# Biogod2020/Spatial-Clip

Hardware: AMD Instinct MI355X
Metric: tile-gene pairs/sec (train step) (higher is better)
Workload: dtype bf16

## Files before the change

### spatial-clip_amd/csrc/sc_gemm8p.hip

```cpp
#include "sc_gemm_common.h"
#include <stdlib.h>
#include <map>
#include <mutex>

namespace {

constexpr int BM = 256, BN = 256, BK = 64;
constexpr int HALF = 128 * 64 * 2;
constexpr int RING = 8 * HALF;
constexpr int EPI_BYTES = 8 * 64 * SC_EPI_LD * 4;
constexpr int LDS_BYTES = EPI_BYTES > RING ? EPI_BYTES : RING;

typedef const __attribute__((address_space(1))) void* gptr_t;
typedef __attribute__((address_space(3))) void* lptr_t;

SC_DEVICE void dma16(const void* src, char* lds_wave_base) {
    __builtin_amdgcn_global_load_lds((gptr_t)src, (lptr_t)lds_wave_base, 16, 0, 0);
}

template <int EPI, bool Q8 = false, bool LUT = false>
SC_DEVICE void epilogue_bf16_lds(f32x4 (&acc)[8][4], const GemmArgs& g, char* strip, int row0, int col0, int lane,
                                 const unsigned* lut = nullptr) {
    float amax_lane = 0.f;
    const float q8s = (Q8 && sc_epi_gelu_fwd(EPI) && g.q8) ? *g.q8_scale : 0.f;
    const int li = lane & 15, lg = lane >> 4;
    constexpr bool kBias = (EPI == SC_EPI_BF16_BIAS || sc_epi_gelu_fwd(EPI));
    f32x4 bj[4];
#pragma unroll
    for (int j = 0; j < 4; ++j) {
        bj[j] = (f32x4){0.f, 0.f, 0.f, 0.f};
        const int c = col0 + j * 16 + lg * 4;
        if (kBias && g.bias && c < g.N) bj[j] = *reinterpret_cast<const f32x4*>(g.bias + c);
    }
    bf16* C = reinterpret_cast<bf16*>(g.C);
    bf16* C2 = reinterpret_cast<bf16*>(g.C2);
    const int rr = lane >> 3, rc = lane & 7;
    const int gcol = col0 + rc * 8;
#pragma unroll
    for (int p = 0; p < 4; ++p) {
#pragma unroll
        for (int ib = 0; ib < 2; ++ib) {
            const int r = ib * 16 + li;
#pragma unroll
            for (int j = 0; j < 4; ++j) {
                const f32x4 v = acc[p * 2 + ib][j] + bj[j];
                const int chunk = (j * 2 + (lg >> 1)) ^ (r & 7);
                *reinterpret_cast<u32x2*>(strip + r * 128 + chunk * 16 + (lg & 1) * 8) = sc_pack4(v[0], v[1], v[2], v[3]);
            }
        }
        __builtin_amdgcn_s_waitcnt(0xC07F);
        __builtin_amdgcn_wave_barrier();
#pragma unroll
        for (int s4 = 0; s4 < 4; ++s4) {
            const int r = s4 * 8 + rr;
            const u32x4 u = *reinterpret_cast<const u32x4*>(strip + r * 128 + ((rc ^ (r & 7)) << 4));
            const int grow = row0 + p * 32 + r;
            if (grow < g.M && gcol < g.N) {
                if (EPI != SC_EPI_GELU_GRAD_PAIR) *reinterpret_cast<u32x4*>(C + (size_t)grow * g.ldc + gcol) = u;
                if (sc_epi_gelu_fwd(EPI)) {
                    union { u32x4 w; bf16x8 h; } x;
                    x.w = u;
                    bf16x8 o;
                    if (EPI == SC_EPI_GELU_PAIR) {
#pragma unroll
                        for (int e = 0; e < 8; ++e) o[e] = (bf16)sc_act((float)x.h[e], g.act);
                    } else {
                        bf16x8 gd;
                        bool formula = true;
                        if (LUT) {
                            unsigned ent[8];
                            bool inside = true;
#pragma unroll
                            for (int e = 0; e < 8; ++e) {
                                const unsigned bits = (u[e >> 1] >> ((e & 1) * 16)) & 0xFFFFu;
                                const unsigned rel = (bits & 0x7FFFu) - (unsigned)SC_GELU_LUT_LO;
                                inside = inside && rel < (unsigned)SC_GELU_LUT_HALF;
                                const unsigned idx = min(rel, (unsigned)SC_GELU_LUT_HALF - 1u) + (bits >> 15) * (unsigned)SC_GELU_LUT_HALF;
                                ent[e] = lut[idx];
                            }
                            formula = __builtin_amdgcn_ballot_w64(!inside) != 0;
                            if (!formula) {
                                union { u32x4 w; bf16x8 h; } lo, hi;
#pragma unroll
                                for (int q = 0; q < 4; ++q) {
                                    lo.w[q] = __builtin_amdgcn_perm(ent[2 * q + 1], ent[2 * q], 0x05040100u);
                                    hi.w[q] = __builtin_amdgcn_perm(ent[2 * q + 1], ent[2 * q], 0x07060302u);
                                }
                                o = lo.h;
                                gd = hi.h;
                            }
                        }
                        if (formula) {
#pragma unroll
                            for (int e = 0; e < 8; ++e) {
                                float hv, gv;
                                sc_act_both((float)x.h[e], g.act, hv, gv);
                                o[e] = (bf16)hv;
                                gd[e] = (bf16)gv;
                            }
                        }
                        *reinterpret_cast<bf16x8*>(C + (size_t)grow * g.ldc + gcol) = gd;
                    }
                    *reinterpret_cast<bf16x8*>(C2 + (size_t)grow * g.ldc2 + gcol) = o;
                    if (Q8 && g.q8) {
                        float r[8];
#pragma unroll
                        for (int e = 0; e < 8; ++e) { r[e] = (float)o[e]; amax_lane = fmaxf(amax_lane, fabsf(r[e])); }
                        *reinterpret_cast<u32x2*>(g.q8 + (size_t)grow * g.ldq8 + gcol) = sc_pack8_fp8(r, q8s);
                    }
                }
            }
        }
        __builtin_amdgcn_s_waitcnt(0xC07F);
        __builtin_amdgcn_wave_barrier();
    }
    if (Q8 && sc_epi_gelu_fwd(EPI) && g.q8) sc_amax_publish(amax_lane, g.q8_amax);
}

constexpr int slot(int D, int q) { return D * 4 * HALF + q * HALF; }

struct Stager {
    const bf16* src[4][2];
    int nt;
    int wave;
};

template <int D, int PH>
SC_DEVICE void phase(char* smem, const Stager& S, int t, const int (&a_off)[2], const int (&b_off)[2], bf16x8 (&a)[8],
                     bf16x8 (&b0)[4], bf16x8 (&b1)[4], f32x4 (&acc)[8][4]) {
    if (PH == 1) {
#pragma unroll
        for (int kk = 0; kk < 2; ++kk)
#pragma unroll
            for (int jj = 0; jj < 2; ++jj)
                b0[kk * 2 + jj] = *reinterpret_cast<const bf16x8*>(smem + slot(D, 1) + b_off[kk] + jj * 2048);
    }
    if (PH == 2) {
#pragma unroll
        for (int kk = 0; kk < 2; ++kk)
#pragma unroll
            for (int jj = 0; jj < 2; ++jj)
                b1[kk * 2 + jj] = *reinterpret_cast<const bf16x8*>(smem + slot(D, 2) + b_off[kk] + jj * 2048);
    }
    if (PH == 1 || PH == 3) {
        constexpr int sl = slot(D, PH == 1 ? 0 : 3);
#pragma unroll
        for (int kk = 0; kk < 2; ++kk)
#pragma unroll
            for (int ii = 0; ii < 4; ++ii)
                a[kk * 4 + ii] = *reinterpret_cast<const bf16x8*>(smem + sl + a_off[kk] + ii * 2048);
    }
    constexpr int q = (PH + 1) & 3;
    constexpr int DS = PH <= 2 ? (D ^ 1) : D;
    const int ts = t + (PH <= 2 ? 1 : 2);
    if (ts < S.nt) {
        dma16(S.src[q][0] + (size_t)ts * BK, smem + slot(DS, q) + S.wave * 1024);
        dma16(S.src[q][1] + (size_t)ts * BK, smem + slot(DS, q) + (8 + S.wave) * 1024);
        asm volatile("s_waitcnt vmcnt(8)" ::: "memory");
    } else {
        asm volatile("s_waitcnt vmcnt(0)" ::: "memory");
    }
    __builtin_amdgcn_sched_barrier(0);
    __builtin_amdgcn_s_barrier();
    __builtin_amdgcn_sched_barrier(0);
    constexpr int mi = PH >= 3 ? 1 : 0;
    constexpr int nj = (PH == 2 || PH == 3) ? 1 : 0;
    __builtin_amdgcn_s_setprio(1);
#pragma unroll
    for (int kk = 0; kk < 2; ++kk)
#pragma unroll
        for (int ii = 0; ii < 4; ++ii)
#pragma unroll
            for (int jj = 0; jj < 2; ++jj)
                acc[mi * 4 + ii][nj * 2 + jj] =
                    sc_mfma16(nj ? b1[kk * 2 + jj] : b0[kk * 2 + jj], a[kk * 4 + ii], acc[mi * 4 + ii][nj * 2 + jj]);
    __builtin_amdgcn_s_setprio(0);
    __builtin_amdgcn_sched_barrier(0);
    __builtin_amdgcn_s_barrier();
    __builtin_amdgcn_sched_barrier(0);
}

template <int D>
SC_DEVICE void ktile(char* smem, const Stager& S, int t, const int (&a_off)[2], const int (&b_off)[2], bf16x8 (&a)[8],
                     bf16x8 (&b0)[4], bf16x8 (&b1)[4], f32x4 (&acc)[8][4]) {
    phase<D, 1>(smem, S, t, a_off, b_off, a, b0, b1, acc);
    phase<D, 2>(smem, S, t, a_off, b_off, a, b0, b1, acc);
    phase<D, 3>(smem, S, t, a_off, b_off, a, b0, b1, acc);
    phase<D, 4>(smem, S, t, a_off, b_off, a, b0, b1, acc);
}

template <int EPI>
__global__ __launch_bounds__(512, 2) void gemm8p_kernel(const GemmArgs g) {
    extern __shared__ __attribute__((aligned(16))) char smem[];
    const int t = threadIdx.x;
    const int lane = t & 63;
    const int wave = __builtin_amdgcn_readfirstlane(t >> 6);
    const int wr = wave >> 2, wc = wave & 3;
    const int li = lane & 15, lg = lane >> 4;

    int idx = sc_xcd_remap(blockIdx.x, gridDim.x);
    int tn, tm, z;
    if (g.col_group > 0) {
        sc_tile_colgroup(idx, g, tm, tn);
        z = 0;
    } else {
        tn = idx % g.ntn;
        idx /= g.ntn;
        tm = idx % g.ntm;
        z = idx / g.ntm;
    }
    const int m0 = tm * BM, n0 = tn * BN;
    const int kbeg = z * g.k_per_split;
    const int kend = min(g.K, kbeg + g.k_per_split);

    Stager S;
    S.nt = (kend - kbeg) / BK;
    S.wave = wave;
#pragma unroll
    for (int p = 0; p < 2; ++p) {
        const int r = (p * 8 + wave) * 8 + (lane >> 3);
        const int lc = (lane & 7) ^ ((r >> 1) & 7);
#pragma unroll
        for (int h = 0; h < 2; ++h) {
            const int ga = min(m0 + (r >> 6) * 128 + h * 64 + (r & 63), g.M - 1);
            const int gb = min(n0 + (r >> 5) * 64 + h * 32 + (r & 31), g.N - 1);
            S.src[h ? 3 : 0][p] = g.A + (size_t)ga * g.lda + kbeg + lc * 8;
            S.src[h ? 2 : 1][p] = g.B + (size_t)gb * g.ldb + kbeg + lc * 8;
        }
    }
    int a_off[2], b_off[2];
#pragma unroll
    for (int kk = 0; kk < 2; ++kk) {
        const int coff = ((kk * 4 + lg) ^ ((li >> 1) & 7)) << 4;
        a_off[kk] = (wr * 64 + li) * 128 + coff;
        b_off[kk] = (wc * 32 + li) * 128 + coff;
    }

    f32x4 acc[8][4];
#pragma unroll
    for (int i = 0; i < 8; ++i)
#pragma unroll
        for (int j = 0; j < 4; ++j) acc[i][j] = (f32x4){0.f, 0.f, 0.f, 0.f};

#pragma unroll
    for (int s = 0; s < 6; ++s) {
        const int ts = s >> 2, q = s & 3;
        if (ts < S.nt) {
            dma16(S.src[q][0] + (size_t)ts * BK, smem + slot(ts & 1, q) + wave * 1024);
            dma16(S.src[q][1] + (size_t)ts * BK, smem + slot(ts & 1, q) + (8 + wave) * 1024);
        }
    }
    if (S.nt > 1) asm volatile("s_waitcnt vmcnt(8)" ::: "memory");
    else asm volatile("s_waitcnt vmcnt(0)" ::: "memory");
    __builtin_amdgcn_sched_barrier(0);
    __builtin_amdgcn_s_barrier();
    if (wr == 1) __builtin_amdgcn_s_barrier();
    __builtin_amdgcn_sched_barrier(0);

    bf16x8 a[8], b0[4], b1[4];
    for (int kt = 0; kt < S.nt; kt += 2) {
        ktile<0>(smem, S, kt, a_off, b_off, a, b0, b1, acc);
        if (kt + 1 < S.nt) ktile<1>(smem, S, kt + 1, a_off, b_off, a, b0, b1, acc);
    }
    if (wr == 0) __builtin_amdgcn_s_barrier();
    asm volatile("s_waitcnt vmcnt(0)" ::: "memory");
    __builtin_amdgcn_sched_barrier(0);

    if (EPI == SC_EPI_GELU_GRAD_PAIR && g.gelu_lut != nullptr) {
        unsigned* lut = reinterpret_cast<unsigned*>(smem + 8 * 4096);
        for (int c = t; c < SC_GELU_LUT_N / 4; c += 512)
            reinterpret_cast<u32x4*>(lut)[c] = reinterpret_cast<const u32x4*>(g.gelu_lut)[c];
        __syncthreads();
        epilogue_bf16_lds<EPI, false, true>(acc, g, smem + wave * 4096, m0 + wr * 128, n0 + wc * 64, lane, lut);
    } else if (EPI == SC_EPI_BF16 || EPI == SC_EPI_BF16_BIAS || sc_epi_gelu_fwd(EPI)) {
        epilogue_bf16_lds<EPI>(acc, g, smem + wave * 4096, m0 + wr * 128, n0 + wc * 64, lane);
    } else {
        const int mw = wr * 128;
        float* ep = reinterpret_cast<float*>(smem) + wave * 64 * SC_EPI_LD;
        EpiRegs<EPI> er;
        sc_epi_load<EPI>(er, m0 + mw, n0 + wc * 64, lane, g, 64);
#pragma unroll
        for (int h = 0; h < 2; ++h) {
#pragma unroll
            for (int i = 0; i < 4; ++i)
#pragma unroll
                for (int j = 0; j < 4; ++j) sc_epi_put(ep, i, j, li, lg, acc[h * 4 + i][j]);
            __builtin_amdgcn_s_waitcnt(0xC07F);
            __builtin_amdgcn_wave_barrier();
            sc_epilogue_store<EPI>(ep, er, m0 + mw + h * 64, n0 + wc * 64, lane, g, z, (h + 1 < 2) ? m0 + mw + 64 : -1, 64);
            __builtin_amdgcn_s_waitcnt(0xC07F);
            __builtin_amdgcn_wave_barrier();
        }
    }
}

__global__ void sc_gelu_lut_fill_kernel(unsigned* lut, int act) {
    const int i = blockIdx.x * blockDim.x + threadIdx.x;
    if (i >= SC_GELU_LUT_N) return;
    const unsigned bits = (unsigned)(SC_GELU_LUT_LO + i % SC_GELU_LUT_HALF) | (i >= SC_GELU_LUT_HALF ? 0x8000u : 0u);
    const float u = __uint_as_float(bits << 16);
    float hv, gv;
    sc_act_both(u, act, hv, gv);
    union { bf16 b; unsigned short s; } h, gq;
    h.b = (bf16)hv;
    gq.b = (bf16)gv;
    lut[i] = ((unsigned)gq.s << 16) | (unsigned)h.s;
}

template <int EPI>
int launch(const GemmArgs& g, int nblocks, hipStream_t st) {
    static bool attr_done = false;
    if (!attr_done) {
        (void)hipFuncSetAttribute(reinterpret_cast<const void*>(&gemm8p_kernel<EPI>),
                                  hipFuncAttributeMaxDynamicSharedMemorySize, LDS_BYTES);
        attr_done = true;
    }
    gemm8p_kernel<EPI><<<nblocks, 512, LDS_BYTES, st>>>(g);
    SC_LAUNCH_CHECK();
    return 1;
}


enum { PW_STEADY = 0, PW_POSTEPI = 1, PW_DRAIN0 = 2 };

struct PStager {
    const bf16* src[4][2];
    long long koff;
    int sk;
    int stile;
    int nt, wave, total, stride;
};

SC_DEVICE void pstage_set_tile(PStager& S, const GemmArgs& g, int lane) {
    const int tn = S.stile % g.ntn, tm = S.stile / g.ntn;
    const int m0 = tm * BM, n0 = tn * BN;
#pragma unroll
    for (int p = 0; p < 2; ++p) {
        const int r = (p * 8 + S.wave) * 8 + (lane >> 3);
        const int lc = (lane & 7) ^ ((r >> 1) & 7);
#pragma unroll
        for (int h = 0; h < 2; ++h) {
            const int ga = min(m0 + (r >> 6) * 128 + h * 64 + (r & 63), g.M - 1);
            const int gb = min(n0 + (r >> 5) * 64 + h * 32 + (r & 31), g.N - 1);
            S.src[h ? 3 : 0][p] = g.A + (size_t)ga * g.lda + lc * 8;
            S.src[h ? 2 : 1][p] = g.B + (size_t)gb * g.ldb + lc * 8;
        }
    }
}
SC_DEVICE void pstage_advance(PStager& S, const GemmArgs& g, int lane) {
    S.sk += 1;
    S.koff += BK;
    if (S.sk == S.nt) {
        S.sk = 0;
        S.koff = 0;
        S.stile += S.stride;
        if (S.stile < S.total) pstage_set_tile(S, g, lane);
    }
}

template <int PH, int ESTORES>
SC_DEVICE void pphase(char* smem, int doff, PStager& S, const GemmArgs& g, int lane, int pw, const int (&a_off)[2],
                      const int (&b_off)[2], bf16x8 (&a)[8], bf16x8 (&b0)[4], bf16x8 (&b1)[4], f32x4 (&acc)[8][4]) {
    const char* cur = smem + doff;
    if (PH == 1) {
#pragma unroll
        for (int kk = 0; kk < 2; ++kk)
#pragma unroll
            for (int jj = 0; jj < 2; ++jj)
                b0[kk * 2 + jj] = *reinterpret_cast<const bf16x8*>(cur + 1 * HALF + b_off[kk] + jj * 2048);
    }
// ... 855 lines not shown
    int total = 0;
    for (int p = 0; p < n; ++p) {
        gg.g[p] = g[p];
        gg.first[p] = total;
        total += g[p].ntm * g[p].ntn * g[p].splitk;
    }
    for (int p = n; p <= SC_WGRAD_GROUP_MAX; ++p) gg.first[p] = total;
    static bool attr_done = false;
    if (!attr_done) {
        (void)hipFuncSetAttribute(reinterpret_cast<const void*>(&gemm8p_tn_group_kernel),
                                  hipFuncAttributeMaxDynamicSharedMemorySize, LDS_BYTES);
        attr_done = true;
    }
    gemm8p_tn_group_kernel<<<total, 512, LDS_BYTES, st>>>(gg);
    SC_LAUNCH_CHECK();
    return 1;
}

int sc_gemm8p_tn_fp8(GemmArgs& g, int splitk_req, float* slabs, hipStream_t st) {
    if (g.M < 256 || g.N < 192 || (g.K % 128) != 0 || (g.M % 16) != 0 || (g.N % 16) != 0) return 0;
    if ((g.lda % 16) != 0 || (g.ldb % 16) != 0) return 0;
    g.ntm = (g.M + BM - 1) / BM;
    g.ntn = (g.N + BN - 1) / BN;
    const int ktiles = g.K / 128;
    int splitk = splitk_req < 1 ? 1 : splitk_req;
    if (slabs == nullptr) splitk = 1;
    if (splitk > ktiles) splitk = ktiles;
    const int tiles_per = (ktiles + splitk - 1) / splitk;
    splitk = (ktiles + tiles_per - 1) / tiles_per;
    g.splitk = splitk;
    g.k_per_split = tiles_per * 128;
    g.slab_stride = 0;
    if (splitk > 1) {
        if (g.ldc != g.N) return 0;
        g.C = slabs;
        g.slab_stride = (long long)g.M * g.N;
    }
    static bool attr_done = false;
    if (!attr_done) {
        (void)hipFuncSetAttribute(reinterpret_cast<const void*>(&gemm8p_tn_f8_kernel), hipFuncAttributeMaxDynamicSharedMemorySize,
                                  LDS_BYTES);
        attr_done = true;
    }
    gemm8p_tn_f8_kernel<<<g.ntm * g.ntn * splitk, 512, LDS_BYTES, st>>>(g);
    SC_LAUNCH_CHECK();
    return 1;
}

static int sc_colgroup_default(int epi, const GemmArgs& g) {
    (void)epi; (void)g;
    return 0;
}

int sc_gemm8p_try(int mode, int epi, GemmArgs& g, int splitk_req, float* slabs, hipStream_t st) {
    if (g.M < 256 || g.N < 192 || (g.K % BK) != 0) return 0;
    if (mode == SC_GEMM_TN && (epi != SC_EPI_F32 || (g.M % 8) != 0 || (g.N % 8) != 0)) return 0;
    if ((long long)g.M * g.N < 256LL * 256 * 8) return 0;
    if (mode == SC_GEMM_NT && splitk_req <= 1) {
        static const int small_tiles = getenv("SC_GEMM_SMALL_TILES") ? atoi(getenv("SC_GEMM_SMALL_TILES")) : 100;
        if ((long long)g.M * g.N < 256LL * 256 * small_tiles) return 0;
    }
    g.ntm = (g.M + BM - 1) / BM;
    g.ntn = (g.N + BN - 1) / BN;
    const int ktiles = g.K / BK;
    int splitk = splitk_req < 1 ? 1 : splitk_req;
    if (epi != SC_EPI_F32 || slabs == nullptr) splitk = 1;
    if (splitk > ktiles) splitk = ktiles;
    int tiles_per = (ktiles + splitk - 1) / splitk;
    splitk = (ktiles + tiles_per - 1) / tiles_per;
    g.splitk = splitk;
    g.k_per_split = tiles_per * BK;
    g.slab_stride = 0;
    if (splitk > 1) {
        if (g.ldc != g.N) return 0;
        g.C = slabs;
        g.slab_stride = (long long)g.M * g.N;
    }
    const int nblocks = g.ntm * g.ntn * splitk;
    if (mode == SC_GEMM_TN) {
        return launch_tn(g, nblocks, st);
    }
    if (epi == SC_EPI_GELU_GRAD_PAIR) {
        const char* sw = getenv("SC_GELU_LUT");
        if (!(sw && sw[0] == '0')) g.gelu_lut = sc_gelu_lut_device(st, g.act);
    }
    static const bool persist = !(getenv("SC_GEMM_PERSIST") && getenv("SC_GEMM_PERSIST")[0] == '0');
    if (g.gelu_lut == nullptr && persist && splitk == 1 && nblocks >= 1024 && ktiles >= 3) {
        if (epi == SC_EPI_BF16) return launch_persistent<SC_EPI_BF16>(g, nblocks, st);
        if (epi == SC_EPI_BF16_BIAS) return launch_persistent<SC_EPI_BF16_BIAS>(g, nblocks, st);
        if (epi == SC_EPI_GELU_PAIR) return launch_persistent<SC_EPI_GELU_PAIR>(g, nblocks, st);
        if (epi == SC_EPI_GELU_GRAD_PAIR) return launch_persistent<SC_EPI_GELU_GRAD_PAIR>(g, nblocks, st);
    }
    g.col_group = 0;
    if (splitk == 1 && g.ntn > 1) {
        int gc = sc_colgroup_default(epi, g);
        if (const char* sw = getenv("SC_GEMM_COLGROUP")) {
            for (const char* p = sw; *p;) {
                char* e = nullptr;
                const long ep = strtol(p, &e, 10);
                if (e == p || *e != ':') break;
                const long v = strtol(e + 1, &e, 10);
                if (ep == epi || ep == -1) gc = (int)v;
                p = (*e == ',') ? e + 1 : e;
                if (*e != ',') break;
            }
        }
        if (gc > 0 && gc < g.ntn) {
            g.col_group = gc;
            g.band_rows = (g.ntm + 7) / 8;
        }
    }
    int rc = 0;
#define SC_CASE(EPI) \
    if (epi == EPI) rc = launch<EPI>(g, nblocks, st);
    SC_CASE(SC_EPI_BF16)
    SC_CASE(SC_EPI_BF16_BIAS)
    SC_CASE(SC_EPI_F32_BIAS_RES)
    SC_CASE(SC_EPI_GELU_PAIR)
    SC_CASE(SC_EPI_BF16_DGELU)
    SC_CASE(SC_EPI_F32)
    SC_CASE(SC_EPI_BF16_BIAS_RES)
    SC_CASE(SC_EPI_GELU_GRAD_PAIR)
    SC_CASE(SC_EPI_BF16_MUL_AUX)
#undef SC_CASE
    return rc;
}

const unsigned* sc_gelu_lut_device(hipStream_t st, int act) {
    static std::mutex mu;
    static std::map<int, unsigned*> all;
    int dev = 0;
    if (hipGetDevice(&dev) != hipSuccess) return nullptr;
    const int key = dev * 2 + (act ? 1 : 0);
    std::lock_guard<std::mutex> lock(mu);
    auto it = all.find(key);
    if (it != all.end()) return it->second;
    unsigned* p = nullptr;
    if (hipMalloc(reinterpret_cast<void**>(&p), SC_GELU_LUT_N * sizeof(unsigned)) != hipSuccess) p = nullptr;
    if (p) {
        sc_gelu_lut_fill_kernel<<<(SC_GELU_LUT_N + 255) / 256, 256, 0, st>>>(p, act ? 1 : 0);
        if (hipGetLastError() != hipSuccess || hipStreamSynchronize(st) != hipSuccess) {
            (void)hipFree(p);
            p = nullptr;
        }
    }
    all[key] = p;
    return p;
}
```

### spatial-clip_amd/csrc/sc_gemm_common.h

```cpp
#pragma once
#include "sc_common.h"
#include "sc_kernels.h"

struct GemmArgs {
    const bf16* A;
    const bf16* B;
    int M, N, K;
    int lda, ldb;
    void* C;
    int ldc;
    void* C2;
    int ldc2;
    const float* bias;
    const float* res;
    int ldres;
    const bf16* aux;
    int ldaux;
    int splitk;
    int k_per_split;
    long long slab_stride;
    int ntm, ntn;
    int tile_offset;
    float* colsum;
    const float* a_scale = nullptr;
    const float* b_scale = nullptr;
    unsigned char* q8 = nullptr;
    long long ldq8 = 0;
    const float* q8_scale = nullptr;
    float* q8_amax = nullptr;
    int a_scale_scalar = 0;
    const unsigned* gelu_lut = nullptr;
    int act = 0;
    int col_group = 0;
    int band_rows = 0;
};

SC_DEVICE void sc_tile_colgroup(int idx, const GemmArgs& g, int& tm, int& tn) {
    const int band_tiles = g.band_rows * g.ntn;
    const int band = idx / band_tiles;
    const int r = idx - band * band_tiles;
    const int row0 = band * g.band_rows;
    const int rows = min(g.band_rows, g.ntm - row0);
    const int nfg = g.ntn / g.col_group;
    const int full = rows * g.col_group * nfg;
    if (r < full) {
        const int gsz = rows * g.col_group;
        const int grp = r / gsz, rr = r - grp * gsz;
        tm = row0 + rr / g.col_group;
        tn = grp * g.col_group + rr % g.col_group;
    } else {
        const int rem = g.ntn - nfg * g.col_group, r2 = r - full;
        tm = row0 + r2 / rem;
        tn = nfg * g.col_group + r2 % rem;
    }
}

constexpr int SC_GELU_LUT_LO = 107 << 7;
constexpr int SC_GELU_LUT_HALF = 25 * 128;
constexpr int SC_GELU_LUT_N = 2 * SC_GELU_LUT_HALF;
const unsigned* sc_gelu_lut_device(hipStream_t st, int act = 0);

constexpr int SC_EPI_LD = 68;

SC_DEVICE void sc_gelu_qe(float x, float& q, float& e) {
    const float y = fabsf(x) * 0.84932180028801904f;
    const float t = __builtin_amdgcn_rcpf(__builtin_fmaf(0.2727374808792225f, y, 1.0f));
    e = __builtin_amdgcn_exp2f(-(y * y));
    float r = __builtin_fmaf(t, 0.5307027145f, -0.7265760135f);
    r = __builtin_fmaf(r, t, 0.7107068705f);
    r = __builtin_fmaf(r, t, -0.142248368f);
    r = __builtin_fmaf(r, t, 0.127414796f);
    q = r * t;
}
SC_DEVICE float sc_gelu_phi(float x, float& e) {
    float q;
    sc_gelu_qe(x, q, e);
    return 0.5f + copysignf(__builtin_fmaf(-q, e, 0.5f), x);
}
SC_DEVICE float sc_gelu_fast(float x) {
    float e;
    return x * sc_gelu_phi(x, e);
}
SC_DEVICE float sc_gelu_grad_fast(float x) {
    float e;
    const float phi = sc_gelu_phi(x, e);
    return __builtin_fmaf(x * e, 0.3989422804014327f, phi);
}
// ... 207 lines not shown
```

### spatial-clip_amd/csrc/sc_kernels.h

```cpp
#pragma once
#include "../../include/spatial_clip_hip.h"

enum sc_attn_path {
    SC_ATTN_PATH_NONE = -1,
    SC_ATTN_FWD_PERSISTENT = 0, SC_ATTN_FWD_PERSISTENT2, SC_ATTN_FWD_PER_HEAD, SC_ATTN_FWD_STREAM,
    SC_ATTN_BWD_CLS = 0, SC_ATTN_BWD_RING, SC_ATTN_BWD_RING8, SC_ATTN_BWD_SINGLE_PASS, SC_ATTN_BWD_PERSISTENT,
    SC_ATTN_BWD_FUSED, SC_ATTN_BWD_DQ_DKV, SC_ATTN_BWD_STREAM
};

extern "C" int sc_debug_attn_last_path(int* fwd, int* bwd);
extern "C" int sc_debug_attn_plan(int B, int L, int H, int dh, int causal, int q_rows, int* fwd, int* bwd);
```

### spatial-clip_amd/ops.py

```python
from __future__ import annotations

import ctypes
from typing import Optional

import torch

from . import _lib
from ._lib import check

NT, TN = 0, 1
(EPI_BF16, EPI_BF16_BIAS, EPI_F32_BIAS_RES, EPI_GELU_PAIR, EPI_BF16_DGELU, EPI_F32, EPI_BF16_BIAS_RES, EPI_GELU_GRAD_PAIR,
 EPI_BF16_MUL_AUX, EPI_QGELU_PAIR, EPI_BF16_DQGELU, EPI_QGELU_GRAD_PAIR) = range(12)


def act_epilogues(quick_gelu: bool):
    if quick_gelu:
        return EPI_QGELU_PAIR, EPI_QGELU_GRAD_PAIR, EPI_BF16_DQGELU
    return EPI_GELU_PAIR, EPI_GELU_GRAD_PAIR, EPI_BF16_DGELU


def _stream() -> int:
    return torch.cuda.current_stream().cuda_stream


# ... 120 lines not shown

def workspace(nfloat: int, device, tag: str = "ws", dtype=torch.float32) -> torch.Tensor:
    key = (device.index, tag, dtype, torch.cuda.current_stream(device).cuda_stream)
    buf = _ws_cache.get(key)
    if buf is None or buf.numel() < nfloat:
        buf = torch.empty(max(int(nfloat), 1024), dtype=dtype, device=device)
        _ws_cache[key] = buf
    return buf


def attn_fwd(qkv: torch.Tensor, B: int, L: int, H: int, dh: int, causal: bool = False,
             out: Optional[torch.Tensor] = None, lse: Optional[torch.Tensor] = None, q_rows: int = 0):
    _req(qkv, torch.bfloat16, "qkv")
    if out is None:
        out = torch.empty((B * L, H * dh), dtype=torch.bfloat16, device=qkv.device)
    if lse is None:
        lse = torch.empty((B, H, L), dtype=torch.float32, device=qkv.device)
    check(_lib.lib().sc_attn_fwd(qkv.data_ptr(), out.data_ptr(), lse.data_ptr(), B, L, H, dh, int(causal), q_rows,
                                 _stream()), "sc_attn_fwd")
    return out, lse


def attn_bwd(qkv, out, dout, lse, B: int, L: int, H: int, dh: int, causal: bool = False,
             dqkv: Optional[torch.Tensor] = None, delta: Optional[torch.Tensor] = None, q_rows: int = 0):
    for t_, n in ((qkv, "qkv"), (out, "out"), (dout, "dout")):
        _req(t_, torch.bfloat16, n)
    if dqkv is None:
        dqkv = torch.empty_like(qkv)
    if delta is None:
        delta = torch.empty((B, H, L), dtype=torch.float32, device=qkv.device)
    check(_lib.lib().sc_attn_bwd(qkv.data_ptr(), out.data_ptr(), dout.data_ptr(), lse.data_ptr(), delta.data_ptr(),
                                 dqkv.data_ptr(), B, L, H, dh, int(causal), q_rows, _stream()), "sc_attn_bwd")
    return dqkv


ATTN_FWD_PATHS = ("persistent", "persistent2", "per_head", "stream")
ATTN_BWD_PATHS = ("cls", "ring", "ring8", "single_pass", "persistent", "fused", "dq_dkv", "stream")


def attn_last_path():
    fn = getattr(_lib.lib(), "sc_debug_attn_last_path")
    fn.restype, fn.argtypes = ctypes.c_int, [ctypes.POINTER(ctypes.c_int)] * 2
    f, b = ctypes.c_int(-1), ctypes.c_int(-1)
    check(fn(ctypes.byref(f), ctypes.byref(b)), "sc_debug_attn_last_path")
    return (ATTN_FWD_PATHS[f.value] if f.value >= 0 else "none", ATTN_BWD_PATHS[b.value] if b.value >= 0 else "none")


def attn_plan(B: int, L: int, H: int, dh: int, causal: bool = False, q_rows: int = 0):
    fn = getattr(_lib.lib(), "sc_debug_attn_plan")
    fn.restype, fn.argtypes = ctypes.c_int, [ctypes.c_int] * 6 + [ctypes.POINTER(ctypes.c_int)] * 2
    f, b = ctypes.c_int(-1), ctypes.c_int(-1)
    check(fn(B, L, H, dh, int(causal), q_rows, ctypes.byref(f), ctypes.byref(b)), "sc_debug_attn_plan")
    return ATTN_FWD_PATHS[f.value], ATTN_BWD_PATHS[b.value]


def _t8_args(t8, rows: int, d: int, what: str):
    buf, scale, amax = t8
    if buf.dtype != torch.uint8 or not buf.is_cuda or buf.stride(-1) != 1 or buf.shape[0] < rows or buf.shape[1] < d:
        raise TypeError(f"{what}: t8 buffer must be a device uint8 matrix of at least [{rows}, {d}]")
    _req(scale, torch.float32, "t8 scale"); _req(amax, torch.float32, "t8 amax")
    if scale.numel() != 1 or amax.numel() != 64:
        raise ValueError(f"{what}: t8 needs a one-element scale and 64 amax slots")
    return buf.data_ptr(), buf.stride(0), scale.data_ptr(), amax.data_ptr()


def layernorm_fwd(x, gamma, beta, y, mean, rstd, rows: int, d: int, ldx: Optional[int] = None,
                  ldy: Optional[int] = None, eps: float = 1e-5, q8: Optional[torch.Tensor] = None,
                  q8_scale_inv: Optional[torch.Tensor] = None, t8=None):
    _req(y, torch.bfloat16, "y")
    if q8 is not None:
        if q8.dtype != torch.uint8 or not q8.is_cuda or q8.stride(-1) != 1:
            raise TypeError("layernorm_fwd: q8 must be a device uint8 matrix")
        _req(q8_scale_inv, torch.float32, "q8_scale_inv")
    if t8 is not None and (x.dtype != torch.bfloat16 or q8 is None):
        raise _lib.SpatialClipHipError("layernorm_fwd: the per-tensor e4m3 copy exists for bf16 rows with the per-row copy (q8)")
    if x.dtype == torch.bfloat16 and t8 is not None:
        tp, tld, tsc, tam = _t8_args(t8, rows, d, "layernorm_fwd")
        check(_lib.lib().sc_layernorm_fwd_x16_t8(x.data_ptr(), ldx if ldx is not None else d, gamma.data_ptr(), beta.data_ptr(),
                                                 y.data_ptr(), ldy if ldy is not None else d, q8.data_ptr(), q8.stride(0),
                                                 q8_scale_inv.data_ptr(), tp, tld, tsc, tam, _ptr(mean), _ptr(rstd), rows, d, eps,
                                                 _stream()), "sc_layernorm_fwd_x16_t8")
        return y
    if x.dtype == torch.bfloat16:
        _req(x, torch.bfloat16, "x")
        check(_lib.lib().sc_layernorm_fwd_x16(x.data_ptr(), ldx if ldx is not None else d, gamma.data_ptr(), beta.data_ptr(),
                                              y.data_ptr(), ldy if ldy is not None else d, _ptr(q8),
                                              q8.stride(0) if q8 is not None else 0, _ptr(q8_scale_inv), _ptr(mean),
                                              _ptr(rstd), rows, d, eps, _stream()), "sc_layernorm_fwd_x16")
        return y
    _req(x, torch.float32, "x")
    if q8 is not None:
        check(_lib.lib().sc_layernorm_fwd_q8(x.data_ptr(), ldx if ldx is not None else d, gamma.data_ptr(),
                                             beta.data_ptr(), y.data_ptr(), ldy if ldy is not None else d, q8.data_ptr(),
                                             q8.stride(0), q8_scale_inv.data_ptr(), _ptr(mean), _ptr(rstd), rows, d, eps,
                                             _stream()), "sc_layernorm_fwd_q8")
        return y
    check(_lib.lib().sc_layernorm_fwd(x.data_ptr(), ldx if ldx is not None else d, gamma.data_ptr(), beta.data_ptr(),
                                      y.data_ptr(), ldy if ldy is not None else d, _ptr(mean), _ptr(rstd), rows, d, eps,
                                      _stream()), "sc_layernorm_fwd")
    return y


def gelu_bf16(u: torch.Tensor, h: torch.Tensor, quick: bool = False) -> torch.Tensor:
    _req(u, torch.bfloat16, "u"); _req(h, torch.bfloat16, "h")
    if not (u.is_contiguous() and h.is_contiguous()) or u.numel() != h.numel():
        raise ValueError("gelu_bf16: contiguous tensors of equal size required")
# ... 467 lines not shown
```

Baseline: 8120.

## Peel last K-tile to prefetch residual and epilogue operands during final MFMAs

Peels the last K-tile of the 8-phase GEMM loop so that, instead of issuing DMA for tiles that do not exist, it loads epilogue operands (aux-mul registers or the bf16 residual) while the final MFMAs run. For the BF16_BIAS_RES epilogue it adds a new variant that loads the residual in two halves and adds it straight into the accumulators. It then reuses the cheaper LDS bf16 bias epilogue rather than the fp32 LDS staging path. This hides the latency of the epilogue global loads behind compute, at the cost of extra registers (the xhalf buffer) and a different rounding order for the residual add. The new path is on by default and can be turned off with an environment variable.

```diff
diff --git a/spatial-clip_amd/csrc/sc_gemm8p.hip b/spatial-clip_amd/csrc/sc_gemm8p.hip
--- a/spatial-clip_amd/csrc/sc_gemm8p.hip
+++ b/spatial-clip_amd/csrc/sc_gemm8p.hip
@@ -117,6 +117,31 @@
     if (Q8 && sc_epi_gelu_fwd(EPI) && g.q8) sc_amax_publish(amax_lane, g.q8_amax);
 }
 
+SC_DEVICE void res_half_load(u32x2 (&raw)[4][4], const GemmArgs& g, int row0, int col0, int li, int lg) {
+    const bf16* res = reinterpret_cast<const bf16*>(g.res);
+#pragma unroll
+    for (int i = 0; i < 4; ++i) {
+        const bf16* rp = res + (size_t)min(row0 + i * 16 + li, g.M - 1) * g.ldres;
+#pragma unroll
+        for (int j = 0; j < 4; ++j) {
+            raw[i][j] = (u32x2){0u, 0u};
+            if (res) raw[i][j] = *reinterpret_cast<const u32x2*>(rp + min(col0 + j * 16 + lg * 4, g.N - 4));
+        }
+    }
+}
+SC_DEVICE void res_half_add(f32x4 (&acc)[8][4], const u32x2 (&raw)[4][4], int half) {
+#pragma unroll
+    for (int i = 0; i < 4; ++i)
+#pragma unroll
+        for (int j = 0; j < 4; ++j) {
+            const u32x2 w = raw[i][j];
+            f32x4& c = acc[half * 4 + i][j];
+            c += (f32x4){__uint_as_float(w[0] << 16), __uint_as_float(w[0] & 0xFFFF0000u), __uint_as_float(w[1] << 16),
+                         __uint_as_float(w[1] & 0xFFFF0000u)};
+            asm volatile("" : "+v"(c));
+        }
+}
+
 constexpr int slot(int D, int q) { return D * 4 * HALF + q * HALF; }
 
 struct Stager {
@@ -125,9 +150,13 @@
     int wave;
 };
 
-template <int D, int PH>
+struct NoEarly {
+    SC_DEVICE void operator()(int) const {}
+};
+
+template <int D, int PH, bool LAST = false, class Early = NoEarly>
 SC_DEVICE void phase(char* smem, const Stager& S, int t, const int (&a_off)[2], const int (&b_off)[2], bf16x8 (&a)[8],
-                     bf16x8 (&b0)[4], bf16x8 (&b1)[4], f32x4 (&acc)[8][4]) {
+                     bf16x8 (&b0)[4], bf16x8 (&b1)[4], f32x4 (&acc)[8][4], const Early& early = Early()) {
     if (PH == 1) {
 #pragma unroll
         for (int kk = 0; kk < 2; ++kk)
@@ -153,7 +182,9 @@
     constexpr int q = (PH + 1) & 3;
     constexpr int DS = PH <= 2 ? (D ^ 1) : D;
     const int ts = t + (PH <= 2 ? 1 : 2);
-    if (ts < S.nt) {
+    if (LAST) {
+        early(PH);
+    } else if (ts < S.nt) {
         dma16(S.src[q][0] + (size_t)ts * BK, smem + slot(DS, q) + S.wave * 1024);
         dma16(S.src[q][1] + (size_t)ts * BK, smem + slot(DS, q) + (8 + S.wave) * 1024);
         asm volatile("s_waitcnt vmcnt(8)" ::: "memory");
@@ -180,16 +211,16 @@
     __builtin_amdgcn_sched_barrier(0);
 }
 
-template <int D>
+template <int D, bool LAST = false, class Early = NoEarly>
 SC_DEVICE void ktile(char* smem, const Stager& S, int t, const int (&a_off)[2], const int (&b_off)[2], bf16x8 (&a)[8],
-                     bf16x8 (&b0)[4], bf16x8 (&b1)[4], f32x4 (&acc)[8][4]) {
-    phase<D, 1>(smem, S, t, a_off, b_off, a, b0, b1, acc);
-    phase<D, 2>(smem, S, t, a_off, b_off, a, b0, b1, acc);
-    phase<D, 3>(smem, S, t, a_off, b_off, a, b0, b1, acc);
-    phase<D, 4>(smem, S, t, a_off, b_off, a, b0, b1, acc);
-}
-
-template <int EPI>
+                     bf16x8 (&b0)[4], bf16x8 (&b1)[4], f32x4 (&acc)[8][4], const Early& early = Early()) {
+    phase<D, 1, LAST>(smem, S, t, a_off, b_off, a, b0, b1, acc, early);
+    phase<D, 2, LAST>(smem, S, t, a_off, b_off, a, b0, b1, acc, early);
+    phase<D, 3, LAST>(smem, S, t, a_off, b_off, a, b0, b1, acc, early);
+    phase<D, 4, LAST>(smem, S, t, a_off, b_off, a, b0, b1, acc, early);
+}
+
+template <int EPI, bool RES_LASTK = false>
 __global__ __launch_bounds__(512, 2) void gemm8p_kernel(const GemmArgs g) {
     extern __shared__ __attribute__((aligned(16))) char smem[];
     const int t = threadIdx.x;
@@ -257,14 +288,33 @@
     if (wr == 1) __builtin_amdgcn_s_barrier();
     __builtin_amdgcn_sched_barrier(0);
 
+    constexpr bool kPeel = sc_epi_aux_mul(EPI) || RES_LASTK;
+    const bool peel = kPeel && S.nt > 1;
+    EpiRegs<EPI> er;
+    u32x2 xhalf[4][4];
+    const int wm0 = m0 + wr * 128, wn0 = n0 + wc * 64;
+    const auto early = [&](int ph) {
+        if constexpr (RES_LASTK) {
+            if (ph == 1) res_half_load(xhalf, g, wm0, wn0, li, lg);
+            if (ph == 3) {
+                res_half_add(acc, xhalf, 0);
+                res_half_load(xhalf, g, wm0 + 64, wn0, li, lg);
+            }
+        } else {
+            if (ph == 1) sc_epi_load<EPI>(er, wm0, wn0, lane, g, 64);
+        }
+    };
+    const int nloop = peel ? S.nt - 1 : S.nt;
     bf16x8 a[8], b0[4], b1[4];
-    for (int kt = 0; kt < S.nt; kt += 2) {
+    for (int kt = 0; kt < nloop; kt += 2) {
         ktile<0>(smem, S, kt, a_off, b_off, a, b0, b1, acc);
-        if (kt + 1 < S.nt) ktile<1>(smem, S, kt + 1, a_off, b_off, a, b0, b1, acc);
-    }
+        if (kt + 1 < nloop) ktile<1>(smem, S, kt + 1, a_off, b_off, a, b0, b1, acc);
+    }
+    if (kPeel && peel) ktile<0, true>(smem + (nloop & 1) * 4 * HALF, S, nloop, a_off, b_off, a, b0, b1, acc, early);
     if (wr == 0) __builtin_amdgcn_s_barrier();
-    asm volatile("s_waitcnt vmcnt(0)" ::: "memory");
-    __builtin_amdgcn_sched_barrier(0);
+    if (!peel) asm volatile("s_waitcnt vmcnt(0)" ::: "memory");
+    __builtin_amdgcn_sched_barrier(0);
+    if constexpr (RES_LASTK) res_half_add(acc, xhalf, 1);
 
     if (EPI == SC_EPI_GELU_GRAD_PAIR && g.gelu_lut != nullptr) {
         unsigned* lut = reinterpret_cast<unsigned*>(smem + 8 * 4096);
@@ -272,13 +322,14 @@
             reinterpret_cast<u32x4*>(lut)[c] = reinterpret_cast<const u32x4*>(g.gelu_lut)[c];
         __syncthreads();
         epilogue_bf16_lds<EPI, false, true>(acc, g, smem + wave * 4096, m0 + wr * 128, n0 + wc * 64, lane, lut);
+    } else if (RES_LASTK) {
+        epilogue_bf16_lds<SC_EPI_BF16_BIAS>(acc, g, smem + wave * 4096, m0 + wr * 128, n0 + wc * 64, lane);
     } else if (EPI == SC_EPI_BF16 || EPI == SC_EPI_BF16_BIAS || sc_epi_gelu_fwd(EPI)) {
         epilogue_bf16_lds<EPI>(acc, g, smem + wave * 4096, m0 + wr * 128, n0 + wc * 64, lane);
     } else {
         const int mw = wr * 128;
         float* ep = reinterpret_cast<float*>(smem) + wave * 64 * SC_EPI_LD;
-        EpiRegs<EPI> er;
-        sc_epi_load<EPI>(er, m0 + mw, n0 + wc * 64, lane, g, 64);
+        if (!peel) early(1);
 #pragma unroll
         for (int h = 0; h < 2; ++h) {
 #pragma unroll
@@ -307,15 +358,15 @@
     lut[i] = ((unsigned)gq.s << 16) | (unsigned)h.s;
 }
 
-template <int EPI>
+template <int EPI, bool RES_LASTK = false>
 int launch(const GemmArgs& g, int nblocks, hipStream_t st) {
     static bool attr_done = false;
     if (!attr_done) {
-        (void)hipFuncSetAttribute(reinterpret_cast<const void*>(&gemm8p_kernel<EPI>),
+        (void)hipFuncSetAttribute(reinterpret_cast<const void*>(&gemm8p_kernel<EPI, RES_LASTK>),
                                   hipFuncAttributeMaxDynamicSharedMemorySize, LDS_BYTES);
         attr_done = true;
     }
-    gemm8p_kernel<EPI><<<nblocks, 512, LDS_BYTES, st>>>(g);
+    gemm8p_kernel<EPI, RES_LASTK><<<nblocks, 512, LDS_BYTES, st>>>(g);
     SC_LAUNCH_CHECK();
     return 1;
 }
@@ -1335,6 +1386,10 @@
             g.band_rows = (g.ntm + 7) / 8;
         }
     }
+    if (epi == SC_EPI_BF16_BIAS_RES && splitk == 1 && ktiles > 1) {
+        const char* sw = getenv("SC_GEMM_RES_INIT");
+        if (!(sw && sw[0] == '0')) return launch<SC_EPI_BF16_BIAS_RES, true>(g, nblocks, st);
+    }
     int rc = 0;
 #define SC_CASE(EPI) \
     if (epi == EPI) rc = launch<EPI>(g, nblocks, st);
```

Result: no change. 8166, median of 6 (+0.6%).

## Split last-wave GEMM tiles into half-height tiles to fill idle CUs

Applied to the files above, without the earlier changes.

When the 256x256 tile count leaves a partial final wave that covers at most half the CUs, those leftover tiles are each split into two 128-row half tiles run by separate blocks. The half-tile path has its own three-stage LDS ring pipeline and a 4x4 accumulator variant of the epilogue. The aim is to cut the tail-wave imbalance where most CUs sit idle while a few finish full tiles. In exchange it adds code paths and a larger LDS request for tail launches, and the half tiles reuse B less.

```diff
diff --git a/spatial-clip_amd/csrc/sc_gemm8p.hip b/spatial-clip_amd/csrc/sc_gemm8p.hip
--- a/spatial-clip_amd/csrc/sc_gemm8p.hip
+++ b/spatial-clip_amd/csrc/sc_gemm8p.hip
@@ -18,8 +18,8 @@
     __builtin_amdgcn_global_load_lds((gptr_t)src, (lptr_t)lds_wave_base, 16, 0, 0);
 }
 
-template <int EPI, bool Q8 = false, bool LUT = false>
-SC_DEVICE void epilogue_bf16_lds(f32x4 (&acc)[8][4], const GemmArgs& g, char* strip, int row0, int col0, int lane,
+template <int EPI, bool Q8 = false, bool LUT = false, int NI = 8>
+SC_DEVICE void epilogue_bf16_lds(f32x4 (&acc)[NI][4], const GemmArgs& g, char* strip, int row0, int col0, int lane,
                                  const unsigned* lut = nullptr) {
     float amax_lane = 0.f;
     const float q8s = (Q8 && sc_epi_gelu_fwd(EPI) && g.q8) ? *g.q8_scale : 0.f;
@@ -37,7 +37,7 @@
     const int rr = lane >> 3, rc = lane & 7;
     const int gcol = col0 + rc * 8;
 #pragma unroll
-    for (int p = 0; p < 4; ++p) {
+    for (int p = 0; p < NI / 2; ++p) {
 #pragma unroll
         for (int ib = 0; ib < 2; ++ib) {
             const int r = ib * 16 + li;
@@ -189,16 +189,178 @@
     phase<D, 4>(smem, S, t, a_off, b_off, a, b0, b1, acc);
 }
 
+constexpr int HRING = 9 * HALF;
+constexpr int hslot(int D, int q) { return (D * 3 + q) * HALF; }
+
+struct HStager {
+    const bf16* src[3][2];
+    int nt;
+    int wave;
+};
+
+template <int D, int PH>
+SC_DEVICE void hphase(char* smem, const HStager& S, int t, const int (&a_off)[2], const int (&b_off)[2], bf16x8 (&a)[8],
+                      bf16x8 (&b0)[4], bf16x8 (&b1)[4], f32x4 (&acc)[4][4]) {
+    if (PH == 1) {
+#pragma unroll
+        for (int kk = 0; kk < 2; ++kk)
+#pragma unroll
+            for (int jj = 0; jj < 2; ++jj)
+                b0[kk * 2 + jj] = *reinterpret_cast<const bf16x8*>(smem + hslot(D, 1) + b_off[kk] + jj * 2048);
+#pragma unroll
+        for (int kk = 0; kk < 2; ++kk)
+#pragma unroll
+            for (int ii = 0; ii < 4; ++ii)
+                a[kk * 4 + ii] = *reinterpret_cast<const bf16x8*>(smem + hslot(D, 0) + a_off[kk] + ii * 2048);
+    } else {
+#pragma unroll
+        for (int kk = 0; kk < 2; ++kk)
+#pragma unroll
+            for (int jj = 0; jj < 2; ++jj)
+                b1[kk * 2 + jj] = *reinterpret_cast<const bf16x8*>(smem + hslot(D, 2) + b_off[kk] + jj * 2048);
+    }
+    constexpr int DS = (D + 2) % 3;
+    const int ts = t + 2;
+    if (ts < S.nt) {
+        if (PH == 1) {
+            dma16(S.src[0][0] + (size_t)ts * BK, smem + hslot(DS, 0) + S.wave * 1024);
+            dma16(S.src[0][1] + (size_t)ts * BK, smem + hslot(DS, 0) + (8 + S.wave) * 1024);
+            dma16(S.src[1][0] + (size_t)ts * BK, smem + hslot(DS, 1) + S.wave * 1024);
+            dma16(S.src[1][1] + (size_t)ts * BK, smem + hslot(DS, 1) + (8 + S.wave) * 1024);
+            asm volatile("s_waitcnt vmcnt(10)" ::: "memory");
+        } else {
+            dma16(S.src[2][0] + (size_t)ts * BK, smem + hslot(DS, 2) + S.wave * 1024);
+            dma16(S.src[2][1] + (size_t)ts * BK, smem + hslot(DS, 2) + (8 + S.wave) * 1024);
+            asm volatile("s_waitcnt vmcnt(8)" ::: "memory");
+        }
+    } else {
+        asm volatile("s_waitcnt vmcnt(0)" ::: "memory");
+    }
+    __builtin_amdgcn_sched_barrier(0);
+    __builtin_amdgcn_s_barrier();
+    __builtin_amdgcn_sched_barrier(0);
+    constexpr int nj = PH - 1;
+    __builtin_amdgcn_s_setprio(1);
+#pragma unroll
+    for (int kk = 0; kk < 2; ++kk)
+#pragma unroll
+        for (int ii = 0; ii < 4; ++ii)
+#pragma unroll
+            for (int jj = 0; jj < 2; ++jj)
+                acc[ii][nj * 2 + jj] = sc_mfma16(nj ? b1[kk * 2 + jj] : b0[kk * 2 + jj], a[kk * 4 + ii], acc[ii][nj * 2 + jj]);
+    __builtin_amdgcn_s_setprio(0);
+    __builtin_amdgcn_sched_barrier(0);
+    __builtin_amdgcn_s_barrier();
+    __builtin_amdgcn_sched_barrier(0);
+}
+
+template <int D>
+SC_DEVICE void hktile(char* smem, const HStager& S, int t, const int (&a_off)[2], const int (&b_off)[2], bf16x8 (&a)[8],
+                      bf16x8 (&b0)[4], bf16x8 (&b1)[4], f32x4 (&acc)[4][4]) {
+    hphase<D, 1>(smem, S, t, a_off, b_off, a, b0, b1, acc);
+    hphase<D, 2>(smem, S, t, a_off, b_off, a, b0, b1, acc);
+}
+
 template <int EPI>
-__global__ __launch_bounds__(512, 2) void gemm8p_kernel(const GemmArgs g) {
-    extern __shared__ __attribute__((aligned(16))) char smem[];
+SC_DEVICE void half_tile(const GemmArgs& g, char* smem, int mh, int n0) {
     const int t = threadIdx.x;
     const int lane = t & 63;
     const int wave = __builtin_amdgcn_readfirstlane(t >> 6);
     const int wr = wave >> 2, wc = wave & 3;
     const int li = lane & 15, lg = lane >> 4;
 
-    int idx = sc_xcd_remap(blockIdx.x, gridDim.x);
+    HStager S;
+    S.nt = g.K / BK;
+    S.wave = wave;
+#pragma unroll
+    for (int p = 0; p < 2; ++p) {
+        const int r = (p * 8 + wave) * 8 + (lane >> 3);
+        const int lc = (lane & 7) ^ ((r >> 1) & 7);
+        const int ga = min(mh + r, g.M - 1);
+        S.src[0][p] = g.A + (size_t)ga * g.lda + lc * 8;
+#pragma unroll
+        for (int h = 0; h < 2; ++h) {
+            const int gb = min(n0 + (r >> 5) * 64 + h * 32 + (r & 31), g.N - 1);
+            S.src[1 + h][p] = g.B + (size_t)gb * g.ldb + lc * 8;
+        }
+    }
+    int a_off[2], b_off[2];
+#pragma unroll
+    for (int kk = 0; kk < 2; ++kk) {
+        const int coff = ((kk * 4 + lg) ^ ((li >> 1) & 7)) << 4;
+        a_off[kk] = (wr * 64 + li) * 128 + coff;
+        b_off[kk] = (wc * 32 + li) * 128 + coff;
+    }
+    f32x4 acc[4][4];
+#pragma unroll
+    for (int i = 0; i < 4; ++i)
+#pragma unroll
+        for (int j = 0; j < 4; ++j) acc[i][j] = (f32x4){0.f, 0.f, 0.f, 0.f};
+
+#pragma unroll
+    for (int s = 0; s < 6; ++s) {
+        const int ts = s / 3, q = s % 3;
+        if (ts < S.nt) {
+            dma16(S.src[q][0] + (size_t)ts * BK, smem + hslot(ts, q) + wave * 1024);
+            dma16(S.src[q][1] + (size_t)ts * BK, smem + hslot(ts, q) + (8 + wave) * 1024);
+        }
+    }
+    if (S.nt > 1) asm volatile("s_waitcnt vmcnt(8)" ::: "memory");
+    else asm volatile("s_waitcnt vmcnt(0)" ::: "memory");
+    __builtin_amdgcn_sched_barrier(0);
+    __builtin_amdgcn_s_barrier();
+    if (wr == 1) __builtin_amdgcn_s_barrier();
+    __builtin_amdgcn_sched_barrier(0);
+
+    bf16x8 a[8], b0[4], b1[4];
+    for (int kt = 0; kt < S.nt; kt += 3) {
+        hktile<0>(smem, S, kt, a_off, b_off, a, b0, b1, acc);
+        if (kt + 1 < S.nt) hktile<1>(smem, S, kt + 1, a_off, b_off, a, b0, b1, acc);
+        if (kt + 2 < S.nt) hktile<2>(smem, S, kt + 2, a_off, b_off, a, b0, b1, acc);
+    }
+    if (wr == 0) __builtin_amdgcn_s_barrier();
+    asm volatile("s_waitcnt vmcnt(0)" ::: "memory");
+    __builtin_amdgcn_sched_barrier(0);
+
+    const int row0 = mh + wr * 64, col0 = n0 + wc * 64;
+    if (EPI == SC_EPI_GELU_GRAD_PAIR && g.gelu_lut != nullptr) {
+        unsigned* lut = reinterpret_cast<unsigned*>(smem + 8 * 4096);
+        for (int c = t; c < SC_GELU_LUT_N / 4; c += 512)
+            reinterpret_cast<u32x4*>(lut)[c] = reinterpret_cast<const u32x4*>(g.gelu_lut)[c];
+        __syncthreads();
+        epilogue_bf16_lds<EPI, false, true>(acc, g, smem + wave * 4096, row0, col0, lane, lut);
+    } else if (EPI == SC_EPI_BF16 || EPI == SC_EPI_BF16_BIAS || sc_epi_gelu_fwd(EPI)) {
+        epilogue_bf16_lds<EPI>(acc, g, smem + wave * 4096, row0, col0, lane);
+    } else {
+        float* ep = reinterpret_cast<float*>(smem) + wave * 64 * SC_EPI_LD;
+        EpiRegs<EPI> er;
+        sc_epi_load<EPI>(er, row0, col0, lane, g, 64);
+#pragma unroll
+        for (int i = 0; i < 4; ++i)
+#pragma unroll
+            for (int j = 0; j < 4; ++j) sc_epi_put(ep, i, j, li, lg, acc[i][j]);
+        __builtin_amdgcn_s_waitcnt(0xC07F);
+        __builtin_amdgcn_wave_barrier();
+        sc_epilogue_store<EPI>(ep, er, row0, col0, lane, g, 0, -1, 64);
+    }
+}
+
+template <int EPI>
+__global__ __launch_bounds__(512, 2) void gemm8p_kernel(const GemmArgs g) {
+    extern __shared__ __attribute__((aligned(16))) char smem[];
+    int idx, hh = -1;
+    if (g.tail_first > 0) {
+        const int b = (int)blockIdx.x - g.tail_first;
+        if (b >= 0) {
+            const int r = sc_xcd_remap(b, 2 * g.tail_rem);
+            idx = g.tail_first + (r >> 1);
+            hh = r & 1;
+        } else {
+            idx = sc_xcd_remap(blockIdx.x, g.tail_first);
+        }
+    } else {
+        idx = sc_xcd_remap(blockIdx.x, gridDim.x);
+    }
     int tn, tm, z;
     if (g.col_group > 0) {
         sc_tile_colgroup(idx, g, tm, tn);
@@ -209,6 +371,17 @@
         tm = idx % g.ntm;
         z = idx / g.ntm;
     }
+    if (hh >= 0) {
+        const int mh = tm * BM + hh * 128;
+        if (mh < g.M) half_tile<EPI>(g, smem, mh, tn * BN);
+        return;
+    }
+    const int t = threadIdx.x;
+    const int lane = t & 63;
+    const int wave = __builtin_amdgcn_readfirstlane(t >> 6);
+    const int wr = wave >> 2, wc = wave & 3;
+    const int li = lane & 15, lg = lane >> 4;
+
     const int m0 = tm * BM, n0 = tn * BN;
     const int kbeg = z * g.k_per_split;
     const int kend = min(g.K, kbeg + g.k_per_split);
@@ -312,10 +485,11 @@
     static bool attr_done = false;
     if (!attr_done) {
         (void)hipFuncSetAttribute(reinterpret_cast<const void*>(&gemm8p_kernel<EPI>),
-                                  hipFuncAttributeMaxDynamicSharedMemorySize, LDS_BYTES);
+                                  hipFuncAttributeMaxDynamicSharedMemorySize, LDS_BYTES > HRING ? LDS_BYTES : HRING);
         attr_done = true;
     }
-    gemm8p_kernel<EPI><<<nblocks, 512, LDS_BYTES, st>>>(g);
+    const int lds = (g.tail_first > 0 && HRING > LDS_BYTES) ? HRING : LDS_BYTES;
+    gemm8p_kernel<EPI><<<nblocks, 512, lds, st>>>(g);
     SC_LAUNCH_CHECK();
     return 1;
 }
@@ -1277,6 +1451,39 @@
     return 0;
 }
 
+extern "C" int sc_debug_gemm_tail_rule(int T, int S, int* nfull, int* rem) {
+    const int r = (S > 0 && T > S) ? T % S : 0;
+    const bool split = r > 0 && 2 * r <= S;
+    if (nfull) *nfull = split ? T - r : T;
+    if (rem) *rem = split ? r : 0;
+    return split ? 1 : 0;
+}
+
+static int sc_last_tail[2] = {-1, -1};
+extern "C" int sc_debug_gemm_last_tail(int* nfull, int* rem, int reset) {
+    if (nfull) *nfull = sc_last_tail[0];
+    if (rem) *rem = sc_last_tail[1];
+    if (reset) sc_last_tail[0] = sc_last_tail[1] = -1;
+    return 0;
+}
+
+static int sc_gemm_slots() {
+    static int cus[64] = {};
+    int dev = 0;
+    if (hipGetDevice(&dev) != hipSuccess || dev < 0 || dev >= 64) return 0;
+    if (cus[dev] == 0) {
+        int n = 0;
+        if (hipDeviceGetAttribute(&n, hipDeviceAttributeMultiprocessorCount, dev) != hipSuccess || n < 1) n = -1;
+        cus[dev] = n;
+    }
+    return cus[dev] > 0 ? cus[dev] : 0;
+}
+
+static bool sc_tail_default(int epi, const GemmArgs& g) {
+    (void)epi; (void)g;
+    return true;
+}
+
 int sc_gemm8p_try(int mode, int epi, GemmArgs& g, int splitk_req, float* slabs, hipStream_t st) {
     if (g.M < 256 || g.N < 192 || (g.K % BK) != 0) return 0;
     if (mode == SC_GEMM_TN && (epi != SC_EPI_F32 || (g.M % 8) != 0 || (g.N % 8) != 0)) return 0;
@@ -1335,9 +1542,23 @@
             g.band_rows = (g.ntm + 7) / 8;
         }
     }
+    g.tail_first = g.tail_rem = 0;
+    int grid = nblocks;
+    if (splitk == 1) {
+        const char* sw = getenv("SC_GEMM_TAIL");
+        const int slots = sw ? atoi(sw) : (sc_tail_default(epi, g) ? sc_gemm_slots() : 0);
+        int nfull = 0, rem = 0;
+        if (slots > 0 && sc_debug_gemm_tail_rule(nblocks, slots, &nfull, &rem)) {
+            g.tail_first = nfull;
+            g.tail_rem = rem;
+            grid = nfull + 2 * rem;
+        }
+    }
+    sc_last_tail[0] = g.tail_first > 0 ? g.tail_first : nblocks;
+    sc_last_tail[1] = g.tail_rem;
     int rc = 0;
 #define SC_CASE(EPI) \
-    if (epi == EPI) rc = launch<EPI>(g, nblocks, st);
+    if (epi == EPI) rc = launch<EPI>(g, grid, st);
     SC_CASE(SC_EPI_BF16)
     SC_CASE(SC_EPI_BF16_BIAS)
     SC_CASE(SC_EPI_F32_BIAS_RES)
diff --git a/spatial-clip_amd/csrc/sc_gemm_common.h b/spatial-clip_amd/csrc/sc_gemm_common.h
--- a/spatial-clip_amd/csrc/sc_gemm_common.h
+++ b/spatial-clip_amd/csrc/sc_gemm_common.h
@@ -33,6 +33,8 @@
     int act = 0;
     int col_group = 0;
     int band_rows = 0;
+    int tail_first = 0;
+    int tail_rem = 0;
 };
 
 SC_DEVICE void sc_tile_colgroup(int idx, const GemmArgs& g, int& tm, int& tn) {
diff --git a/spatial-clip_amd/csrc/sc_kernels.h b/spatial-clip_amd/csrc/sc_kernels.h
--- a/spatial-clip_amd/csrc/sc_kernels.h
+++ b/spatial-clip_amd/csrc/sc_kernels.h
@@ -10,3 +10,5 @@
 
 extern "C" int sc_debug_attn_last_path(int* fwd, int* bwd);
 extern "C" int sc_debug_attn_plan(int B, int L, int H, int dh, int causal, int q_rows, int* fwd, int* bwd);
+extern "C" int sc_debug_gemm_tail_rule(int T, int S, int* nfull, int* rem);
+extern "C" int sc_debug_gemm_last_tail(int* nfull, int* rem, int reset);
diff --git a/spatial-clip_amd/ops.py b/spatial-clip_amd/ops.py
--- a/spatial-clip_amd/ops.py
+++ b/spatial-clip_amd/ops.py
@@ -196,6 +196,23 @@
     f, b = ctypes.c_int(-1), ctypes.c_int(-1)
     check(fn(B, L, H, dh, int(causal), q_rows, ctypes.byref(f), ctypes.byref(b)), "sc_debug_attn_plan")
     return ATTN_FWD_PATHS[f.value], ATTN_BWD_PATHS[b.value]
+
+
+def gemm_tail_rule(T: int, S: int):
+    fn = getattr(_lib.lib(), "sc_debug_gemm_tail_rule")
+    fn.restype, fn.argtypes = ctypes.c_int, [ctypes.c_int] * 2 + [ctypes.POINTER(ctypes.c_int)] * 2
+    nfull, rem = ctypes.c_int(-1), ctypes.c_int(-1)
+    split = fn(T, S, ctypes.byref(nfull), ctypes.byref(rem))
+    assert bool(split) == (rem.value > 0)
+    return nfull.value, rem.value
+
+
+def gemm_last_tail(reset: bool = False):
+    fn = getattr(_lib.lib(), "sc_debug_gemm_last_tail")
+    fn.restype, fn.argtypes = ctypes.c_int, [ctypes.POINTER(ctypes.c_int)] * 2 + [ctypes.c_int]
+    nfull, rem = ctypes.c_int(-1), ctypes.c_int(-1)
+    fn(ctypes.byref(nfull), ctypes.byref(rem), int(reset))
+    return nfull.value, rem.value
 
 
 def _t8_args(t8, rows: int, d: int, what: str):
```

Result: faster. 8077 before, 8201 after, median of 6 (+1.5%).
